# una-dinosauria/local-search-quantization

Hardware: AMD Instinct MI355X
Metric: vectors encoded/sec (ICM, m=8 h=256) (higher is better)
Workload: dtype f32

## Files before the change

local-search-quantization_amd/csrc/lsq_icmq.hip:

```cpp
#include <stdlib.h>

#include <type_traits>

#include <atomic>

#include "lsq_q16.h"
#include "lsq_xload.h"
#ifndef LSQ_WALKQ_PRIO_SHIPPED
#define LSQ_WALKQ_PRIO_SHIPPED 1
#endif
#ifdef LSQ_TUNING
__device__ unsigned long long *g_walkq_dbg = nullptr;
__device__ unsigned int g_walkq_dbg_slot = 0;
__device__ unsigned long long *g_walkq_dbg_cur = nullptr;
__device__ unsigned long long *g_walkq_blk = nullptr;
#define LSQ_WALKQ_DBG_WAVE0 (24 + 2 * 65)
#define LSQ_WALKQ_DBG_WORDS (LSQ_WALKQ_DBG_WAVE0 + 16)
#define DBG_STAMP(k) do { if (dbgp && threadIdx.x == 0) dbgp[k] = wall_clock64(); } while (0)
#define DBG_WAVE_STAMP(w) do { if (dbgp && (threadIdx.x & 63) == 0) dbgp[LSQ_WALKQ_DBG_WAVE0 + (w)] = wall_clock64(); } while (0)
#define LSQ_WALKQ_PRIO_MODE(abl) ((abl) >> 16)
#else
#define DBG_STAMP(k) do {} while (0)
#define LSQ_WALKQ_PRIO_MODE(abl) LSQ_WALKQ_PRIO_SHIPPED
#endif
// ... 217 lines not shown
        for (int k = 0; k < m; ++k) {
            if (k == j) continue;
            const double tr = (double)trange[(j * m + k) * 3] * (1.0 + 1e-6), tm = (double)trange[(j * m + k) * 3 + 1], gm = (double)trange[(j * m + k) * 3 + 2];
            rsum += tr;
            tsum += tm;
            Gmax += gm;
            sub += 2.0 * (tm + gm) + tr;
        }
        const double smax = W + sigmax + Gmax + tsum;
        sub += (W + Gmax + sigmax) * 3.0 + 2.0 * Gmax;
        const double D = rsum / 65500.0;
        const double eps = (double)(m + 1) * smax * 5.9604644775390625e-8 * 2.0 + sub * 5.9604644775390625e-8 * 2.0;
        const double slack = (double)m * (0.5 + 1.0 / 32.0) * D + eps + 65535.0 * D * 2.384185791015625e-7;
        nd.D = (float)D;
        nd.invD = (float)(1.0 / D);
        nd.hiq = (float)fmin(floor((hiU - loU) / D), 65535.0);
        nd.slack = slack;
        const double w = 2.0 * slack / D;
        nd.window = (w < 30000.0) ? (int)w + 1 : 65535;
        if (!(D > 1e-30 && D < 1e30 && rsum == rsum && smax < 1e30)) ok = false;
        if (!(nd.invD > 1e-30f && nd.invD < 1e30f)) ok = false;
        P->node[j] = nd;
    }
    P->ok = ok ? 1 : 0;
    P->nflag = 0;
}

template <int SLQ>
__global__ __launch_bounds__(256) void tables_to_q16_slices_kernel(const float *__restrict__ T, uint16_t *__restrict__ Tq, int m,
                                                                   const lsq_q16_params *__restrict__ P, const float *__restrict__ rowmin,
                                                                   const float *__restrict__ colmean) {
    constexpr int NS = LSQ_H / SLQ, LPV = SLQ / 8;
    const int64_t total = (int64_t)m * NS * (m - 1) * LSQ_H * LPV;
    const int64_t e = (int64_t)blockIdx.x * 256 + threadIdx.x;
    if (e >= total) return;
    const int qq = (int)(e % LPV);
    int64_t r = e / LPV;
    const int b = (int)(r % LSQ_H); r /= LSQ_H;
    const int kk = (int)(r % (m - 1)); r /= (m - 1);
    const int slice = (int)(r % NS);
    const int j = (int)(r / NS);
    const int k = kk + (kk >= j ? 1 : 0);
    const float lo = rowmin[((int64_t)j * m + k) * LSQ_H + b], inv = P->node[j].invD;
    const float *src = T + (((int64_t)j * m + k) * LSQ_H + b) * LSQ_H + slice * SLQ + qq * 8;
    const float *gs = colmean + ((int64_t)j * m + k) * LSQ_H + slice * SLQ + qq * 8;
    uint32_t w[4];
#pragma unroll
    for (int t = 0; t < 4; ++t) {
        const float q0 = fminf(fmaxf(rintf(((src[2 * t] - gs[2 * t]) - lo) * inv), 0.0f), 65535.0f);
        const float q1 = fminf(fmaxf(rintf(((src[2 * t + 1] - gs[2 * t + 1]) - lo) * inv), 0.0f), 65535.0f);
        w[t] = (uint32_t)q0 | ((uint32_t)q1 << 16);
    }
    const int64_t dst = (((int64_t)j * NS + slice) * (m - 1) * LSQ_H + q16_row_index<SLQ>(m, kk, b)) * LPV + qq;
    reinterpret_cast<u32x4 *>(Tq)[dst] = (u32x4){w[0], w[1], w[2], w[3]};
}

template <int M>
__device__ inline int q16_refine(const float *__restrict__ U, const uint16_t *__restrict__ Uq, const uint16_t *__restrict__ Tq,
                                 const float *__restrict__ T, uint8_t *__restrict__ rec, unsigned short *__restrict__ valid,
                                 const uint8_t *__restrict__ ref_rec, const unsigned short *__restrict__ ref_valid, int64_t n, int j,
                                 int64_t lo, const unsigned short *list, const uint32_t *arec, int namb, int SLF, int abl, unsigned short *vmir) {
    using RT = WalkqRot<M>;
    constexpr int CS = (M <= 8) ? 8 : 16;
    constexpr int RW = CS / 4;
    constexpr int AREC = 2 + RW;
    if (abl & 4) return 0;
    constexpr int NS = LSQ_H / RT::SLQ;
    constexpr int TAB = (M - 1) * LSQ_H * (RT::SLQ / 8);
    constexpr int NW = RT::NT / 64;
    const int lane = threadIdx.x & 63, wave = threadIdx.x >> 6;
    const int grp = lane >> 4, t16 = lane & 15;
    const int sl = (16 * t16) / RT::SLQ, off = (16 * t16) % RT::SLQ;
    const uint16_t *__restrict__ Uqj = Uq + (int64_t)j * n * LSQ_H;
    const uint16_t *__restrict__ Tqj = Tq + ((int64_t)j * NS + sl) * TAB * 8 + off;
    const float *__restrict__ Tj = T + (int64_t)j * M * LSQ_H * LSQ_H;
    const bool have_ref = ref_rec && ref_valid;
    int nexact = 0;
    for (int r0 = wave * 4; r0 < namb; r0 += NW * 4) {
        const int r = r0 + grp;
        const bool act = r < namb;
        const uint32_t *ar = arec + (act ? r : r0) * AREC;
        const uint32_t key = ar[0], limit = ar[1];
        uint32_t rw[RW];
#pragma unroll
        for (int w2 = 0; w2 < RW; ++w2) rw[w2] = ar[2 + w2];
        const int ci = (int)(key & 0xffffu), a1 = (int)((key >> 16) & 0xffu), a2 = (int)(key >> 24);
        const int64_t i = lo + (RT::LHOLE ? list[((ci >> 4) << 7) + (ci & 15)] : list[ci]);
        const u32x4 *up = reinterpret_cast<const u32x4 *>(Uqj + ((int64_t)sl * n + ((abl & 2) ? (int64_t)0 : i)) * RT::SLQ + off);
        u32x4 s0 = (u32x4){0xffffffffu, 0xffffffffu, 0xffffffffu, 0xffffffffu}, s1 = s0;
        if (!(abl & 8)) { s0 = up[0]; s1 = up[1]; }
        unsigned short vo = 0, rv = 0;
        uint32_t rr[RW];
#pragma unroll
        for (int w2 = 0; w2 < RW; ++w2) rr[w2] = 0;
        if (t16 == 0) {
            if (valid) vo = valid[i];
            if (have_ref) {
#pragma unroll
                for (int w2 = 0; w2 < RW; ++w2) rr[w2] = reinterpret_cast<const uint32_t *>(ref_rec + i * CS)[w2];
                rv = ref_valid[i];
            }
        }
        float term = 0.0f;
        if (M <= 8) {
            const int cand = (t16 < 8) ? a1 : a2, tt = t16 & 7;
            if (abl & 1) term = 1.0f;
            else if (tt == 0) term = U[(int64_t)j * n * LSQ_H + ((int64_t)(cand / SLF) * n + ((abl & 16) ? lo : i)) * SLF + (cand % SLF)];
            else if (tt < M) {
                const int k = (tt - 1) + ((tt - 1) >= j ? 1 : 0);
                const uint32_t bk = (rw[k >> 2] >> (8 * (k & 3))) & 0xffu;
                term = Tj[((int64_t)(k * LSQ_H) + bk) * LSQ_H + cand];
            }
        }
#pragma unroll
        for (int kk = 0; kk < M - 1; ++kk) {
            if (abl & 8) break;
            const int k = kk + (kk >= j ? 1 : 0);
            const uint32_t bk = (rw[k >> 2] >> (8 * (k & 3))) & 0xffu;
            const u32x4 *tp = reinterpret_cast<const u32x4 *>(Tqj + (int64_t)q16_row_index<RT::SLQ>(M, kk, (int)bk) * RT::SLQ);
            const u32x4 b0 = tp[0], b1 = tp[1];
            s0.x = pk_add_u16(s0.x, b0.x); s0.y = pk_add_u16(s0.y, b0.y); s0.z = pk_add_u16(s0.z, b0.z); s0.w = pk_add_u16(s0.w, b0.w);
            s1.x = pk_add_u16(s1.x, b1.x); s1.y = pk_add_u16(s1.y, b1.y); s1.z = pk_add_u16(s1.z, b1.z); s1.w = pk_add_u16(s1.w, b1.w);
        }
        uint32_t mask = 0;
#define LSQ_SURV(W, B) mask |= (((W) & 0xffffu) <= limit ? 1u : 0u) << (B); mask |= (((W) >> 16) <= limit ? 1u : 0u) << ((B) + 1);
        LSQ_SURV(s0.x, 0) LSQ_SURV(s0.y, 2) LSQ_SURV(s0.z, 4) LSQ_SURV(s0.w, 6) LSQ_SURV(s1.x, 8) LSQ_SURV(s1.y, 10) LSQ_SURV(s1.z, 12) LSQ_SURV(s1.w, 14)
#undef LSQ_SURV
        if (!act) mask = 0;
        float bv = __builtin_inff();
        int bi = 0x7fffffff;
        if (M <= 8) {
            float e = __shfl(term, (lane & ~7), 64);
#pragma unroll
            for (int q = 1; q < M; ++q) e = e + __shfl(term, (lane & ~7) + q, 64);
            const float e1 = __shfl(e, lane & ~15, 64), e2 = __shfl(e, (lane & ~15) + 8, 64);
            if (a1 / 16 == t16) mask &= ~(1u << (a1 % 16));
            if (a2 / 16 == t16) mask &= ~(1u << (a2 % 16));
            bv = e1; bi = a1;
            if (e2 < bv || (e2 == bv && a2 < bi)) { bv = e2; bi = a2; }
            if (act && t16 == 0) nexact += 2;
        }
        while (mask) {
            const int a = 16 * t16 + __builtin_ctz(mask);
            mask &= mask - 1;
            const float ev = q16_exact_value<M, RW>(U, T, n, SLF, j, i, rw, a);
            ++nexact;
            if (ev < bv || (ev == bv && a < bi)) { bv = ev; bi = a; }
        }
#pragma unroll
        for (int o = 8; o > 0; o >>= 1) {
            const float ov = __shfl_xor(bv, o, 16);
            const int oi = __shfl_xor(bi, o, 16);
            if (ov < bv || (ov == bv && oi < bi)) { bv = ov; bi = oi; }
        }
        if (act && t16 == 0) {
            const uint8_t c8 = (uint8_t)bi;
            const uint8_t old = (uint8_t)(rw[j >> 2] >> (8 * (j & 3)));
            if (c8 != old) store_code<CS>(rec, i, j, c8, rw);
            if (valid) {
                unsigned short vm = (c8 != old) ? (unsigned short)(1u << j) : (unsigned short)(vo | (1u << j));
                if (have_ref) {
                    bool same = true;
#pragma unroll
                    for (int w2 = 0; w2 < RW; ++w2) {
                        uint32_t mine = rw[w2];
                        if (w2 == (j >> 2)) mine = (mine & ~(0xffu << (8 * (j & 3)))) | ((uint32_t)c8 << (8 * (j & 3)));
                        same = same && (mine == rr[w2]);
                    }
                    if (same) vm = (unsigned short)(vm | rv);
                }
                valid[i] = vm;
                if (vmir) vmir[i - lo] = vm;
            }
        }
    }
    return nexact;
}

constexpr int WALKQ_MISC_BYTES = (20 + LSQ_WALK_COUNTERS) * 4;

template <int M>
__global__ __launch_bounds__(WalkqRot<M>::NT) __attribute__((amdgpu_waves_per_eu(4, 4))) void icm_walkq_kernel(const float *__restrict__ U, const uint16_t *__restrict__ Uq, const uint16_t *__restrict__ Tq,
                                                       const float *__restrict__ T, uint8_t *__restrict__ rec, unsigned short *__restrict__ valid,
                                                       int64_t n, const WalkNodes nodes, int per_pass, int use_skip, int direct_max,
                                                       unsigned long long *__restrict__ active_total,
                                                       const uint8_t *__restrict__ ref_rec, const unsigned short *__restrict__ ref_valid,
                                                       const lsq_q16_params *__restrict__ P, int SLF, const unsigned short *__restrict__ qflag, int abl,
                                                       const unsigned *__restrict__ gate) {
    using RT = WalkqRot<M>;
    constexpr int CS = (M <= 8) ? 8 : 16;
    constexpr int NS = LSQ_H / RT::SLQ;
    constexpr int LPV = RT::SLQ / 8;
    constexpr int VPW = 64 / LPV;
    constexpr int CW = (M - 1 + 3) / 4;
    constexpr int RW = CS / 4;
    constexpr int TAB = (M - 1) * LSQ_H * LPV;
    constexpr int PP = RT::pp();
    if (P->ok == 0) return;
    if (gate && *gate != 2u) return;
    extern __shared__ u32x4 lds_walkq[];
    constexpr int MAIN_BYTES = RT::lds_bytes();
    int *misc = reinterpret_cast<int *>(reinterpret_cast<char *>(lds_walkq) + MAIN_BYTES);
#ifdef LSQ_TUNING
    unsigned long long *dbgp = nullptr;
    if (g_walkq_dbg) {
        unsigned &dbg_slot_s = reinterpret_cast<unsigned *>(misc)[19];
        if (threadIdx.x == 0) dbg_slot_s = (blockIdx.x == 0) ? atomicAdd(&g_walkq_dbg_slot, 1u) : 0u;
        __syncthreads();
        if (blockIdx.x == 0 && dbg_slot_s < 4096) dbgp = g_walkq_dbg + (size_t)dbg_slot_s * LSQ_WALKQ_DBG_WORDS;
    }
    DBG_STAMP(0);
    if (blockIdx.x == 0 && threadIdx.x == 0) g_walkq_dbg_cur = dbgp;
    if (g_walkq_blk && threadIdx.x == 0) g_walkq_blk[2 * blockIdx.x] = wall_clock64();
#endif
    if ((uint32_t)(uintptr_t)(lds_char *)lds_walkq != 0u) __builtin_trap();
    if (LSQ_WALKQ_PRIO_MODE(abl) & 4) __builtin_amdgcn_s_setprio(3);
    u32x4 *tab = lds_walkq;
    constexpr bool HOLE = RT::HOLE;
    constexpr bool LHOLE = RT::LHOLE;
    constexpr bool ROT8 = M <= 8, ROT16 = M > 8;
    constexpr int TABE = RT::TAB_BYTES / 16;
    uint32_t *bestA = HOLE ? reinterpret_cast<uint32_t *>(reinterpret_cast<char *>(lds_walkq) + RT::HOLE_BYTE0)
                           : reinterpret_cast<uint32_t *>(lds_walkq + TABE);
    uint32_t *bestB = HOLE ? reinterpret_cast<uint32_t *>(lds_walkq + TABE) : bestA + PP;
    unsigned short *list = LHOLE ? reinterpret_cast<unsigned short *>(reinterpret_cast<char *>(lds_walkq) + RT::HOLE_BYTE0)
                                 : reinterpret_cast<unsigned short *>(bestB + PP);
    auto listp = [&](int i) -> unsigned short * { return LHOLE ? list + ((i >> 4) << 7) + (i & 15) : list + i; };
    constexpr bool MIRROR = RT::mirror();
    auto keyA = [&](int ci) -> uint32_t * { return HOLE ? bestA + ((ci >> 4) << 6) + (ci & 15) : bestA + ci; };
    auto f32slot = [&](int i) -> unsigned short * { return reinterpret_cast<unsigned short *>(keyA(i >> 1)) + (i & 1); };
    unsigned short *vmir = (MIRROR && valid) ? list + PP : nullptr;
    int *wave_tot = misc;
    int &nact_s = misc[16];
    int &redo_s = misc[17];
    int &f32_s = misc[18];
    unsigned *stat_s = reinterpret_cast<unsigned *>(misc) + 20;
    for (int e = threadIdx.x; e < LSQ_WALK_COUNTERS; e += RT::NT) stat_s[e] = 0u;
    __syncthreads();

    const int lane = threadIdx.x & 63;
    const int wave = __builtin_amdgcn_readfirstlane((int)(threadIdx.x >> 6));
    const int v = lane / LPV, q = lane % LPV;
    constexpr int NW = RT::NT / 64;
    constexpr int EPT = 4096 / RT::NT;
    constexpr int step = NW * VPW;

    struct Item { u32x4 u; uint32_t r[RW]; };

    auto walk_slices = [&](const int j, const int64_t lo, const int nact, const bool dense) {
#ifndef LSQ_TUNING
        unsigned long long *dbgp = nullptr; (void)dbgp;
#endif
        const uint16_t *__restrict__ Uqj = Uq + (int64_t)j * n * LSQ_H;
        const uint16_t *__restrict__ Tqj = Tq + (int64_t)j * NS * TAB * 8;
        uint32_t sel[CW > 0 ? CW : 1];
#pragma unroll
        for (int w = 0; w < CW; ++w) {
            uint32_t sv = 0;
#pragma unroll
            for (int t = 0; t < 4; ++t) {
                const int kk = 4 * w + t;
                const int k = kk + (kk >= j ? 1 : 0);
                sv |= (uint32_t)((kk < M - 1 ? k - 4 * w : 0) & 7) << (8 * t);
            }
            sel[w] = sv;
        }
        constexpr int NST = (TAB + RT::NT - 1) / RT::NT;
        u32x4 nxt[NST > 0 ? NST : 1];
        uint32_t selC0 = 0x0c0c0c0cu, selC1 = 0x0c0c0c0cu, base0 = 0u, base1 = 0x01000000u;
        uint32_t rotA = 0x0c0c0c0cu, rotB = 0x0c0c0c0cu, rot1A = 0x0c0c0c0cu, rot1B = 0x0c0c0c0cu, b0a = 0u, b0b = 0u, b1a = 0u, b1b = 0u;
        if constexpr (ROT16) {
#pragma unroll
            for (int t = 0; t < 8; ++t) {
                if (t < RT::NT0) {
                    const uint32_t slot = (uint32_t)(t + v) % (uint32_t)RT::NT0;
                    const uint32_t ab = ((slot << 5) | ((uint32_t)q << 4)) << (8 * (t & 3));
                    if (t < 4) { rotA = (rotA & ~(0xffu << (8 * t))) | (slot << (8 * t)); b0a |= ab; }
                    else { rotB = (rotB & ~(0xffu << (8 * (t - 4)))) | (slot << (8 * (t - 4))); b0b |= ab; }
                }
                if (t < RT::NT1) {
                    const uint32_t slot = (uint32_t)(t + v) % (uint32_t)(RT::NT1 ? RT::NT1 : 1);
                    const uint32_t ab = ((slot << 5) + (((uint32_t)q + 1u) << 4)) << (8 * (t & 3));
                    if (t < 4) { rot1A = (rot1A & ~(0xffu << (8 * t))) | (slot << (8 * t)); b1a |= ab; }
                    else { rot1B = (rot1B & ~(0xffu << (8 * (t - 4)))) | (slot << (8 * (t - 4))); b1b |= ab; }
                }
            }
        }
        if constexpr (ROT8) {
#pragma unroll
            for (int t = 0; t < RT::NT0; ++t) {
                const uint32_t slot = (uint32_t)(t + v) % (uint32_t)(RT::NT0 ? RT::NT0 : 1);
                const uint32_t k = slot + (slot >= (uint32_t)j ? 1u : 0u);
                selC0 = (selC0 & ~(0xffu << (8 * t))) | (k << (8 * t));
                base0 |= ((slot << 6) | ((uint32_t)q << 4)) << (8 * t);
            }
#pragma unroll
            for (int t = 0; t < RT::NT1; ++t) {
                const uint32_t slot = (uint32_t)(t + v) % (uint32_t)(RT::NT1 ? RT::NT1 : 1);
                const uint32_t k = 4u + slot + (4u + slot >= (uint32_t)j ? 1u : 0u);
                selC1 = (selC1 & ~(0xffu << (8 * t))) | (k << (8 * t));
                base1 |= ((slot << 6) | ((uint32_t)q << 4)) << (8 * t);
            }
        }
        const uint32_t v4 = (uint32_t)v * 4u;
        constexpr uint32_t LIST_BYTE0 = (uint32_t)(LHOLE ? 0 : RT::TAB_BYTES + PP * RT::KEY_BYTES);
        const int limv = q == 0 ? nact - v : -0x7fffffff;
        auto rot_entry = [&](auto R_) -> int {
            constexpr int r = decltype(R_)::value;
            constexpr int g = r * RT::NT >= RT::G0_ENTRIES ? 1 : 0, nt = g ? RT::NT1 : RT::NT0, e0 = r * RT::NT - g * RT::G0_ENTRIES;
            const int eg = e0 + (int)threadIdx.x;
            if constexpr (nt == RT::SPL) return g * 4096 + eg;
            else { const int code = eg / (RT::EPS * (nt ? nt : 1)); return g * 4096 + code * 16 + (eg - code * RT::EPS * nt); }
        };
        auto prefetch_tab = [&](int sl) {
            const u32x4 *src = reinterpret_cast<const u32x4 *>(Tqj) + (int64_t)sl * TAB;
#pragma unroll
            for (int r = 0; r < NST; ++r) {
                const int e = (int)threadIdx.x + r * RT::NT;
                nxt[r] = (e < TAB) ? src[e] : (u32x4){0u, 0u, 0u, 0u};
            }
        };
        prefetch_tab(0);
        const int prio = LSQ_WALKQ_PRIO_MODE(abl);
        const int wslot = (prio & 8) ? NW - 1 - wave : wave;
        const int ipw = (wslot * VPW < nact) ? (nact - wslot * VPW + step - 1) / step : 0;
        const int ipw_u = (prio & 3) ? __builtin_amdgcn_readfirstlane(ipw) : 0;
        const int h1 = (ipw_u + 3) >> 2, h2 = (ipw_u + 1) >> 1, h3 = (3 * ipw_u + 3) >> 2;
        auto item_prio = [&](int t) {
            const int tu = __builtin_amdgcn_readfirstlane(t);
            if ((prio & 3) == 1 || (prio & 3) == 3) {
                if (tu < h1) __builtin_amdgcn_s_setprio(3);
                else if (tu < h2) __builtin_amdgcn_s_setprio(2);
                else if (tu < h3) __builtin_amdgcn_s_setprio(1);
                else __builtin_amdgcn_s_setprio(0);
            } else if ((prio & 3) == 2) {
                if (tu < h2) __builtin_amdgcn_s_setprio(1);
                else __builtin_amdgcn_s_setprio(0);
            } else if (prio & 4) __builtin_amdgcn_s_setprio(0);
        };
        auto fixed_prio = [&]() {
            if (prio & 4) __builtin_amdgcn_s_setprio(3);
            else if (prio & 3) __builtin_amdgcn_s_setprio(0);
        };
        int ls = 0, lit = 0;
        const char *ub = reinterpret_cast<const char *>(Uqj + lo * RT::SLQ);
        const char *const rb = reinterpret_cast<const char *>(rec + lo * CS);
        const int64_t plane_bytes = n * (int64_t)(RT::SLQ * 2);
        auto load_next = [&](Item &it) {
            int ci = wslot * VPW + lit * step + v;
            ci = ci < nact ? ci : nact - 1;
            uint32_t li = (uint32_t)ci;
            if (!dense) {
                if constexpr (!LHOLE) li = *reinterpret_cast<lds_u16 *>(LIST_BYTE0 + 2u * (uint32_t)ci);
                else li = *listp(ci);
            }
#ifdef LSQ_TUNING
            const uint32_t uo = ((abl & 32) ? (li & 63u) : li) * (uint32_t)(RT::SLQ * 2) + (uint32_t)q * 16u;
#else
            const uint32_t uo = li * (uint32_t)(RT::SLQ * 2) + (uint32_t)q * 16u;
#endif
            it.u = __builtin_nontemporal_load(reinterpret_cast<const u32x4 *>(ub + uo));
#ifdef LSQ_TUNING
            const uint32_t *rp = reinterpret_cast<const uint32_t *>(rb + ((abl & 512) ? (li & 63u) : li) * (uint32_t)CS);
#else
            const uint32_t *rp = reinterpret_cast<const uint32_t *>(rb + li * (uint32_t)CS);
#endif
#pragma unroll
            for (int w = 0; w < RW; ++w) it.r[w] = rp[w];
            if (++lit >= ipw) {
                lit = 0;
                if (++ls < NS) ub += plane_bytes;
            }
        };
        auto compute = [&](const Item &cur, int slice, int c0) {
            u32x4 s = cur.u;
            if constexpr (ROT16) {
                uint32_t dw[4] = {0u, 0u, 0u, 0u};
#pragma unroll
                for (int w = 0; w < CW; ++w) dw[w] = __builtin_amdgcn_perm((w + 1 < RW) ? cur.r[w + 1] : 0u, cur.r[w], sel[w]);
                const uint32_t cw4[4] = {__builtin_amdgcn_perm(dw[1], dw[0], rotA), __builtin_amdgcn_perm(dw[1], dw[0], rotB),
                                         __builtin_amdgcn_perm(dw[3], dw[2], rot1A), __builtin_amdgcn_perm(dw[3], dw[2], rot1B)};
                const uint32_t bw4[4] = {b0a, b0b, b1a, b1b};
#pragma unroll
                for (int g4 = 0; g4 < 4; ++g4) {
                    const int cnt = g4 < 2 ? (RT::NT0 - 4 * g4 < 4 ? RT::NT0 - 4 * g4 : 4) : (RT::NT1 - 4 * (g4 - 2) < 4 ? RT::NT1 - 4 * (g4 - 2) : 4);
                    if (cnt <= 0) continue;
                    u32x4 rd[4];
#pragma unroll
                    for (int t = 0; t < 4; ++t)
                        if (t < cnt) {
                            const uint32_t a = __builtin_amdgcn_perm(cw4[g4], bw4[g4], 0x0c0c0400u + 0x0101u * (uint32_t)t);
                            rd[t] = *reinterpret_cast<lds_cu32x4 *>(a + (g4 < 2 ? 0u : 0xfff0u));
                        }
#ifdef LSQ_TUNING
                    if (!(abl & 64))
#endif
                    {
#pragma unroll
                        for (int t = 0; t < 4; t += 2) {
                            if (t + 1 < cnt) {
                                s.x = s.x + rd[t].x + rd[t + 1].x; s.y = s.y + rd[t].y + rd[t + 1].y;
                                s.z = s.z + rd[t].z + rd[t + 1].z; s.w = s.w + rd[t].w + rd[t + 1].w;
                            } else if (t < cnt) {
                                s.x += rd[t].x; s.y += rd[t].y; s.z += rd[t].z; s.w += rd[t].w;
                            }
                        }
                    }
                    if (g4 < 3) asm volatile("" : "+v"(s.x), "+v"(s.y), "+v"(s.z), "+v"(s.w) : : "memory");
                }
            } else {
                u32x4 rd[M > 1 ? M - 1 : 1];
                const uint32_t c0r = __builtin_amdgcn_perm(cur.r[1], cur.r[0], selC0);
#pragma unroll
                for (int t = 0; t < RT::NT0; ++t)
                    rd[t] = *reinterpret_cast<lds_cu32x4 *>(__builtin_amdgcn_perm(c0r, base0, 0x0c0c0400u + 0x0101u * (uint32_t)t));
                auto add_rows = [&](int k0, int k1) {
#ifdef LSQ_TUNING
                    if (abl & 64) return;
#endif
#pragma unroll
                    for (int kk = k0; kk < k1; kk += 2) {
                        if (kk + 1 < k1) {
                            s.x = s.x + rd[kk].x + rd[kk + 1 < M - 1 ? kk + 1 : kk].x; s.y = s.y + rd[kk].y + rd[kk + 1 < M - 1 ? kk + 1 : kk].y;
                            s.z = s.z + rd[kk].z + rd[kk + 1 < M - 1 ? kk + 1 : kk].z; s.w = s.w + rd[kk].w + rd[kk + 1 < M - 1 ? kk + 1 : kk].w;
                        } else {
                            s.x += rd[kk].x; s.y += rd[kk].y; s.z += rd[kk].z; s.w += rd[kk].w;
                        }
                    }
                };
                if constexpr (RT::NT1 > 0) {
                    const uint32_t c1r = __builtin_amdgcn_perm(cur.r[1], cur.r[0], selC1);
                    add_rows(0, RT::NT0);
                    asm volatile("" : "+v"(s.x), "+v"(s.y), "+v"(s.z), "+v"(s.w) : : "memory");
#pragma unroll
                    for (int t = 0; t < RT::NT1; ++t)
                        rd[RT::NT0 + t] = *reinterpret_cast<lds_cu32x4 *>(__builtin_amdgcn_perm(c1r, base1, 0x0c030400u + 0x0101u * (uint32_t)t));
                    add_rows(RT::NT0, M - 1);
                } else add_rows(0, M - 1);
            }
#ifdef LSQ_TUNING
            if (abl & 128) {
                if ((q == 0) & (c0 + v < nact) & (s.x == 0x12345678u)) *keyA(c0 + v) = s.y ^ s.z;
                return;
            }
#endif
            constexpr uint32_t HI = 0xffff0000u;
            const uint32_t k0 = s.x << 16, k1 = (s.x & HI) | 1u;
            const uint32_t k2 = (s.y << 16) | 2u, k3 = (s.y & HI) | 3u;
            const uint32_t k4 = (s.z << 16) | 4u, k5 = (s.z & HI) | 5u;
            const uint32_t k6 = (s.w << 16) | 6u, k7 = (s.w & HI) | 7u;
            const uint32_t lc = umin(k6, k7), hc = umax(k6, k7);
            uint32_t l0 = umin3(k0, k1, k2), h0 = umed3(k0, k1, k2);
            const uint32_t lb = umin3(k3, k4, k5), hb = umed3(k3, k4, k5);
            top2_merge(l0, h0, lb, hb);
            top2_merge(l0, h0, lc, hc);
            const uint32_t base = (uint32_t)(RT::SLQ * slice) + 8u * (uint32_t)q;
            l0 += base; h0 += base;
            if (LPV >= 2) top2_merge(l0, h0, dpp_u32<DPP_XOR1>(l0), dpp_u32<DPP_XOR1>(h0));
            if (LPV >= 4) top2_merge(l0, h0, dpp_u32<DPP_XOR2>(l0), dpp_u32<DPP_XOR2>(h0));
            if (c0 < limv) {
                if constexpr (HOLE) {
                    const uint32_t sA = (uint32_t)__builtin_amdgcn_readfirstlane((int)((uint32_t)RT::HOLE_BYTE0 + (uint32_t)c0 * 16u));
                    const uint32_t sB = (uint32_t)__builtin_amdgcn_readfirstlane((int)((uint32_t)RT::TAB_BYTES + (uint32_t)c0 * 4u));
                    const uint32_t old = __hip_atomic_fetch_min(reinterpret_cast<lds_u32 *>(sA + v4), l0, __ATOMIC_RELAXED, __HIP_MEMORY_SCOPE_WORKGROUP);
                    __hip_atomic_fetch_min(reinterpret_cast<lds_u32 *>(sB + v4), umin(umax(old, l0), h0), __ATOMIC_RELAXED, __HIP_MEMORY_SCOPE_WORKGROUP);
                } else {
                    const uint32_t old = atomicMin(&bestA[c0 + v], l0);
                    atomicMin(&bestB[c0 + v], umin(umax(old, l0), h0));
                }
            }
        };
        Item buf[RT::DEPTH];
#pragma unroll
        for (int e = 0; e < RT::DEPTH; ++e) load_next(buf[e]);
        int phase = 0;
        for (int slice = 0; slice < NS; ++slice) {
            __syncthreads();
#ifdef LSQ_TUNING
            if (slice < 8) DBG_STAMP(3 + slice);
#endif
            static_for<NST>([&](auto R_) {
                constexpr int r = decltype(R_)::value;
                if ((r + 1) * RT::NT <= TAB || r * RT::NT + (int)threadIdx.x < TAB) tab[rot_entry(R_)] = nxt[r];
            });
            __syncthreads();
#ifdef LSQ_TUNING
            if (slice == 4) DBG_STAMP(20);
#endif
            if (slice + 1 < NS) prefetch_tab(slice + 1);
#ifdef LSQ_TUNING
            if (slice == 4) DBG_STAMP(21);
#endif
            int c0 = wslot * VPW, t = 0;
            auto run = [&](auto P_) {
                constexpr int PH = decltype(P_)::value;
                for (; t + RT::DEPTH <= ipw; t += RT::DEPTH) {
                    if ((prio & 3) != 3) item_prio(t);
#pragma unroll
                    for (int e = 0; e < RT::DEPTH; ++e) {
                        if ((prio & 3) == 3) item_prio(t + e);
                        compute(buf[(PH + e) % RT::DEPTH], slice, c0); load_next(buf[(PH + e) % RT::DEPTH]); c0 += step;
                    }
                }
#pragma unroll
                for (int e = 0; e < RT::DEPTH - 1; ++e)
                    if (t < ipw) {
                        item_prio(t);
                        compute(buf[(PH + e) % RT::DEPTH], slice, c0); load_next(buf[(PH + e) % RT::DEPTH]); c0 += step;
                        ++t; phase = (PH + e + 1) % RT::DEPTH;
                    }
            };
            bool ran = false;
            auto try_phase = [&](auto P_) {
                if constexpr (decltype(P_)::value < RT::DEPTH) {
                    if (!ran && phase == decltype(P_)::value) { run(P_); ran = true; }
                }
            };
            try_phase(std::integral_constant<int, 0>{}); try_phase(std::integral_constant<int, 1>{});
            try_phase(std::integral_constant<int, 2>{}); try_phase(std::integral_constant<int, 3>{});
            fixed_prio();
#ifdef LSQ_TUNING
            if (slice == 4) { DBG_STAMP(22); DBG_WAVE_STAMP(wave); }
#endif
        }
        __syncthreads();
    };

    constexpr int LB = LSQ_LIGHT_LB(M);
    int64_t lo_cur = 0;
    auto light_list = [&](const int j, const int count, auto pick) {
        const float *__restrict__ Usj = U + (int64_t)j * n * LSQ_H;
        const float *__restrict__ Tj = T + (int64_t)j * M * LSQ_H * LSQ_H;
        for (int r0 = wave; r0 < count; r0 += NW * LB) {
            int64_t vi[LB];
            bool on[LB];
#pragma unroll
            for (int e = 0; e < LB; ++e) {
                const int r = r0 + e * NW;
                on[e] = r < count;
                vi[e] = lo_cur + __builtin_amdgcn_readfirstlane((int)pick(on[e] ? r : r0));
            }
            light_update<M, CS, LB>(rec, valid, ref_rec, ref_valid, Usj, Tj, n, SLF, j, vi, on, lane, vmir, lo_cur);
        }
    };

    const int64_t npass = (n + per_pass - 1) / per_pass;
    for (int64_t pass = blockIdx.x; pass < npass; pass += gridDim.x) {
        const int64_t lo = pass * per_pass;
        const int64_t hi = (lo + per_pass < n) ? lo + per_pass : n;
        const int cnt = (int)(hi - lo);
        lo_cur = lo;
        if (vmir) {
            __syncthreads();
            for (int idx = (int)threadIdx.x; idx < cnt; idx += RT::NT) vmir[idx] = valid[lo + idx];
            __syncthreads();
        }
        for (int nu = 0; nu < nodes.count; ++nu) {
            const int j = nodes.j[nu];
            int tix = (int)threadIdx.x;
            asm volatile("" : "+v"(tix));
#ifdef LSQ_TUNING
            if (dbgp && threadIdx.x == 0 && pass == (int64_t)blockIdx.x && nu < 64) dbgp[24 + nu] = wall_clock64();
#endif
            {
                const int base = tix * EPT;
                int f[EPT], c = 0;
#pragma unroll
                for (int e = 0; e < EPT; ++e) {
                    const int idx = base + e;
                    f[e] = 0;
                    if (idx < cnt) f[e] = (!use_skip) || !(((vmir ? vmir[idx] : valid[lo + idx]) >> j) & 1);
                    c += f[e];
                }
                int inc = c;
#pragma unroll
                for (int off = 1; off < 64; off <<= 1) {
                    const int t = __shfl_up(inc, off, 64);
                    if (lane >= off) inc += t;
                }
                if (lane == 63) wave_tot[wave] = inc;
                DBG_STAMP(16);
                __syncthreads();
                DBG_STAMP(17);
                int wbase = 0;
                for (int w2 = 0; w2 < wave; ++w2) wbase += wave_tot[w2];
                int pos = wbase + inc - c;
#pragma unroll
                for (int e = 0; e < EPT; ++e)
                    if (f[e]) *listp(pos++) = (unsigned short)(base + e);
                if (threadIdx.x == RT::NT - 1) { nact_s = wbase + inc; redo_s = 0; f32_s = 0; }
                DBG_STAMP(18);
                __syncthreads();
            }
            const int nact = nact_s;
            DBG_STAMP(1);
#ifdef LSQ_TUNING
            if (dbgp && threadIdx.x == 0 && pass == (int64_t)blockIdx.x && nu < 64) dbgp[24 + 65 + nu] = (unsigned long long)nact;
#endif
            if (nact == 0) { __syncthreads(); continue; }
            if (threadIdx.x == 0) {
                stat_s[0] += (unsigned)nact;
                stat_s[nact <= direct_max ? 2 : 3] += 1u;
                stat_s[4 + ((nodes.pos0 + nu) & (LSQ_WALK_TRACE - 1))] += (unsigned)nact;
            }
            if (nact <= direct_max) {
                light_list(j, nact, [&](int r) { return *listp(r); });
                __syncthreads();
                continue;
            }
            for (int ci = tix; ci < nact; ci += RT::NT) { *keyA(ci) = 0xffffffffu; bestB[ci] = 0xffffffffu; }
            DBG_STAMP(2);
            walk_slices(j, lo, nact, nact == cnt);
            DBG_STAMP(11);
            const lsq_q16_node &nd = P->node[j];
            const int window = nd.window;
            constexpr int EPD = (PP + RT::NT - 1) / RT::NT;
            constexpr int AREC = 2 + RW;
            constexpr int ACAP = (PP * 4) / (AREC * 4);
            {
                int64_t vi[EPD];
                uint32_t vcode[EPD], vkey[EPD], vlim[EPD];
                bool von[EPD], vamb[EPD], vf32[EPD];
                constexpr bool ONE_TRIP = (M <= 8);
                uint32_t rw[EPD][RW], rr[EPD][RW];
                unsigned short vo[EPD], rv[EPD], fl[EPD];
                uint32_t kA[EPD], kB[EPD];
                const bool have_ref = ref_rec && ref_valid;
#pragma unroll
                for (int e = 0; e < EPD; ++e) {
                    const int ci = tix + e * RT::NT;
                    vi[e] = lo; kA[e] = 0; kB[e] = 0; vo[e] = 0; rv[e] = 0; fl[e] = 0;
#pragma unroll
                    for (int w2 = 0; w2 < RW; ++w2) { rw[e][w2] = 0; rr[e][w2] = 0; }
                    if (ci < nact) {
                        kA[e] = *keyA(ci); kB[e] = bestB[ci];
                        vi[e] = lo + *listp(ci);
                        fl[e] = qflag[vi[e]];
                        if constexpr (ONE_TRIP) {
#pragma unroll
                            for (int w2 = 0; w2 < RW; ++w2) rw[e][w2] = reinterpret_cast<const uint32_t *>(rec + vi[e] * CS)[w2];
                            if (valid) vo[e] = valid[vi[e]];
                            if (have_ref) {
#pragma unroll
                                for (int w2 = 0; w2 < RW; ++w2) rr[e][w2] = reinterpret_cast<const uint32_t *>(ref_rec + vi[e] * CS)[w2];
                                rv[e] = ref_valid[vi[e]];
                            }
                        }
                    }
                }
#pragma unroll
                for (int e = 0; e < EPD; ++e) {
                    const int ci = tix + e * RT::NT;
                    von[e] = false; vamb[e] = false; vf32[e] = false; vcode[e] = 0; vkey[e] = 0; vlim[e] = 0;
                    if (ci < nact) {
                        vcode[e] = kA[e] & 0xffffu;
                        vkey[e] = (uint32_t)ci | ((kA[e] & 0xffu) << 16) | ((kB[e] & 0xffu) << 24);
                        vlim[e] = (kA[e] >> 16) + (uint32_t)window;
                        vf32[e] = (fl[e] >> j) & 1;
                        vamb[e] = !vf32[e] && ((int)(kB[e] >> 16) - (int)(kA[e] >> 16) <= window);
                        von[e] = !vamb[e] && !vf32[e];
                    }
                    if constexpr (!ONE_TRIP) {
                        if (von[e] || vamb[e]) {
#pragma unroll
                            for (int w2 = 0; w2 < RW; ++w2) rw[e][w2] = reinterpret_cast<const uint32_t *>(rec + vi[e] * CS)[w2];
                        }
                        if (von[e]) {
                            if (valid) vo[e] = valid[vi[e]];
                            if (have_ref) {
#pragma unroll
                                for (int w2 = 0; w2 < RW; ++w2) rr[e][w2] = reinterpret_cast<const uint32_t *>(ref_rec + vi[e] * CS)[w2];
                                rv[e] = ref_valid[vi[e]];
                            }
                        }
                    }
                }
                __syncthreads();
                uint32_t *arec = bestB;
#pragma unroll
                for (int e = 0; e < EPD; ++e) {
                    if (von[e]) {
                        const uint8_t c8 = (uint8_t)vcode[e];
                        const uint8_t old = (uint8_t)(rw[e][j >> 2] >> (8 * (j & 3)));
                        if (c8 != old) store_code<CS>(rec, vi[e], j, c8, rw[e]);
                        if (valid) {
                            unsigned short vm = (c8 != old) ? (unsigned short)(1u << j) : (unsigned short)(vo[e] | (1u << j));
                            if (have_ref) {
                                bool same = true;
#pragma unroll
                                for (int w2 = 0; w2 < RW; ++w2) {
                                    uint32_t mine = rw[e][w2];
                                    if (w2 == (j >> 2)) mine = (mine & ~(0xffu << (8 * (j & 3)))) | ((uint32_t)c8 << (8 * (j & 3)));
                                    same = same && (mine == rr[e][w2]);
                                }
                                if (same) vm = (unsigned short)(vm | rv[e]);
                            }
                            valid[vi[e]] = vm;
                            if (vmir) vmir[vi[e] - lo] = vm;
                        }
                    }
                    bool tof32 = vf32[e];
                    if (vamb[e]) {
                        const int slot = atomicAdd(&redo_s, 1);
                        if (slot < ACAP) {
                            arec[slot * AREC] = vkey[e];
                            arec[slot * AREC + 1] = vlim[e];
#pragma unroll
                            for (int w2 = 0; w2 < RW; ++w2) arec[slot * AREC + 2 + w2] = rw[e][w2];
                        } else tof32 = true;
                    }
                    if (tof32) *f32slot(atomicAdd(&f32_s, 1)) = (unsigned short)(vkey[e] & 0xffffu);
                }
            }
            __syncthreads();
            DBG_STAMP(12);
            const int namb = redo_s < ACAP ? redo_s : ACAP;
            int nexact = q16_refine<M>(U, Uq, Tq, T, rec, valid, ref_rec, ref_valid, n, j, lo, list, bestB, namb, SLF, abl, vmir);
            {
                const int nf32 = f32_s;
                light_list(j, nf32, [&](int r) { return *listp(*f32slot(r)); });
                if (threadIdx.x == 0 && nf32) atomicAdd(&stat_s[4 + LSQ_WALK_TRACE + 2], (unsigned)nf32);
            }
            {
#pragma unroll
                for (int o = 32; o > 0; o >>= 1) nexact += __shfl_xor(nexact, o, 64);
                if (lane == 0 && nexact) atomicAdd(&stat_s[4 + LSQ_WALK_TRACE + 1], (unsigned)nexact);
                if (threadIdx.x == 0 && namb) atomicAdd(&stat_s[4 + LSQ_WALK_TRACE], (unsigned)namb);
            }
            __syncthreads();
            DBG_STAMP(13);
#ifdef LSQ_TUNING
            if (dbgp && threadIdx.x == 0) { dbgp[14] = (unsigned long long)nact; dbgp[15] = (unsigned long long)namb; }
#endif
        }
    }
    __syncthreads();
#ifdef LSQ_TUNING
    if (dbgp && threadIdx.x == 0) dbgp[24 + 64] = wall_clock64();
    if (g_walkq_blk && threadIdx.x == 0) g_walkq_blk[2 * blockIdx.x + 1] = wall_clock64();
#endif
    if (active_total)
        for (int e = threadIdx.x; e < LSQ_WALK_COUNTERS; e += RT::NT)
            if (stat_s[e]) atomicAdd(active_total + e, (unsigned long long)stat_s[e]);
}

}

#ifdef LSQ_TUNING
extern "C" __attribute__((visibility("default"))) int lsq_tuning_set_walkq_debug(void *buf) {
    unsigned zero = 0;
    LSQ_HIP(hipMemcpyToSymbol(HIP_SYMBOL(g_walkq_dbg), &buf, sizeof(buf)));
    LSQ_HIP(hipMemcpyToSymbol(HIP_SYMBOL(g_walkq_dbg_slot), &zero, sizeof(zero)));
    return LSQ_OK;
}
extern "C" __attribute__((visibility("default"))) int lsq_tuning_set_walkq_block_clock(void *buf) {
    LSQ_HIP(hipMemcpyToSymbol(HIP_SYMBOL(g_walkq_blk), &buf, sizeof(buf)));
    return LSQ_OK;
}
#endif

__global__ void q16_road_kernel(const lsq_q16_params *__restrict__ P, unsigned *__restrict__ road, long long pairs, long long fallback_div) {
    if (threadIdx.x != 0) return;
    const bool filtered = P->ok == 1 && (long long)P->nflag * fallback_div <= pairs;
    road[0] = filtered ? 2u : 0u;
    if (!filtered) road[1] += 1u;
}
__global__ void q16_probe_kernel(const unsigned long long *__restrict__ probe, unsigned long long *__restrict__ totals, unsigned *__restrict__ road,
                                 unsigned long long probe_div) {
    const int e = threadIdx.x;
    if (e < LSQ_WALK_COUNTERS && totals) totals[e] += probe[e];
    if (e == 0 && road[0] == 2u && probe_div > 0) {
        const unsigned long long hard = probe[4 + LSQ_WALK_TRACE] + probe[4 + LSQ_WALK_TRACE + 2];
        if ((double)hard * (double)probe_div > (double)probe[0]) { road[0] = 0u; road[1] += 1u; }
    }
}
int lsq_launch_q16_road(hipStream_t s, const lsq_q16_params *P, unsigned *road, int64_t pairs, int64_t fallback_div) {
    hipLaunchKernelGGL(q16_road_kernel, dim3(1), dim3(64), 0, s, P, road, (long long)pairs, (long long)fallback_div);
    LSQ_HIP(hipGetLastError());
    return LSQ_OK;
}
int lsq_launch_q16_probe(hipStream_t s, const unsigned long long *probe, unsigned long long *totals, unsigned *road, int64_t probe_div) {
    hipLaunchKernelGGL(q16_probe_kernel, dim3(1), dim3(128), 0, s, probe, totals, road, (unsigned long long)probe_div);
    LSQ_HIP(hipGetLastError());
    return LSQ_OK;
}

const void *lsq_probe_kernel_icmq() { return reinterpret_cast<const void *>(&q16_range_init_kernel); }

template <class XT>
int lsq_launch_unary_shift_panel(hipStream_t s, const XT *Xp, int64_t rows, int d, int m, const lsq_q16_work &w, int64_t row0) {
    if (rows <= 0) return LSQ_OK;
    const int64_t shift_blocks = (rows * 16 + 255) / 256;
    LSQ_SHIFT_LAUNCH(d, dim3((unsigned)(shift_blocks < 2048 ? shift_blocks : 2048)), s, Xp, w.means, rows, d, m, w.sigma + (size_t)row0 * m,
                       &w.qrange[lsq_q16_work::Q_PANEL_SINK], &w.qrange[lsq_q16_work::Q_SIGBOUND], w.qflag, row0, w.P);
    LSQ_HIP(hipGetLastError());
    return LSQ_OK;
}

template int lsq_launch_unary_shift_panel(hipStream_t, const float *, int64_t, int, int, const lsq_q16_work &, int64_t);
template int lsq_launch_unary_shift_panel(hipStream_t, const uint8_t *, int64_t, int, int, const lsq_q16_work &, int64_t);

int lsq_q16_sample_rows(int64_t n, int d, int64_t *rts_out) {
    const int64_t nsample = d <= 128 ? 16384 : (d <= 512 ? 8192 : 4096);
    const int64_t rts = n > nsample ? n / nsample : 1;
    if (rts_out) *rts_out = rts;
    return (int)((n + 128 * rts - 1) / (128 * rts));
}

template <class XT>
int lsq_launch_q16_prepare(hipStream_t s, const XT *X, int64_t n, int d, const float *K, const float *sci, const float *T, int m, const lsq_q16_work &w,
                           int tables_changed) {
    using W = lsq_q16_work;
    const XT *Xsample = static_cast<const XT *>(w.Xsample);
    unsigned *sigmax = &w.qrange[W::Q_SIGMAX];
    static_assert(W::Q_SIGBOUND == W::Q_SIGMAX + 1 && W::Q_WORDS == 2 * LSQ_MAX_M + 4, "q16_params_kernel's sigrange[0 .. 1], q16_range_init_kernel's fill");
    if (tables_changed) {
        LSQ_HIP(hipMemsetAsync(w.bad, 0, sizeof(int), s));
        hipLaunchKernelGGL(table_colmean_kernel, dim3((unsigned)(m * m)), dim3(256), 0, s, T, m, w.colmean);
        hipLaunchKernelGGL(unary_colshift_kernel, dim3((unsigned)m), dim3(256), 0, s, w.colmean, m, w.colshift);
        if (m > 1) hipLaunchKernelGGL(table_range_kernel, dim3((unsigned)(m * m)), dim3(256), 0, s, T, m, w.colmean, w.trange, w.rowmin, w.bad);
        hipLaunchKernelGGL(codebook_means_kernel, dim3((unsigned)((d + 63) / 64), (unsigned)m), dim3(256), 0, s, K, m, d, w.means);
    }
    hipLaunchKernelGGL(q16_range_init_kernel, dim3(1), dim3(64), 0, s, w.qrange, m);
    lsq_gemm_q16 range;
    range.qrange = w.qrange; range.colshift = w.colshift;
    if (Xsample) {
        const int64_t shift_blocks = (w.nsample_rows * 16 + 255) / 256;
        LSQ_SHIFT_LAUNCH(d, dim3((unsigned)(shift_blocks < 2048 ? shift_blocks : 2048)), s, Xsample, w.means, w.nsample_rows, d, m, w.sigma_sample, sigmax);
        range.sigma = w.sigma_sample;
        LSQ_TRY(lsq_launch_chain_gemm(s, Xsample, K, sci, -2.0f, w.nsample_rows, m * LSQ_H, d, LSQ_H, 0, 0, nullptr, 0, w.nsample_rows, 0, &range));
        LSQ_HIP(hipMemsetAsync(w.qflag, 0, sizeof(unsigned short) * (size_t)((n + 1) & ~(int64_t)1), s));
    } else if (n > 0) {
        const int64_t shift_blocks = (n * 16 + 255) / 256;
        LSQ_SHIFT_LAUNCH(d, dim3((unsigned)(shift_blocks < 2048 ? shift_blocks : 2048)), s, X, w.means, n, d, m, w.sigma, sigmax);
        int64_t rts64 = 1;
        (void)lsq_q16_sample_rows(n, d, &rts64);
        range.rts = (int)rts64; range.sigma = w.sigma;
        LSQ_TRY(lsq_launch_chain_gemm(s, X, K, sci, -2.0f, n, m * LSQ_H, d, LSQ_H, 0, 0, nullptr, 0, n, 0, &range));
        LSQ_HIP(hipMemsetAsync(w.qflag, 0, sizeof(unsigned short) * (size_t)((n + 1) & ~(int64_t)1), s));
    }
    hipLaunchKernelGGL(q16_params_kernel, dim3(1), dim3(64), 0, s, w.trange, w.bad, w.qrange, m, w.P, sigmax, Xsample ? 2.0f : 1.0f);
    if (m > 1) {
        const int slq = lsq_q16_slice_width(m);
        const int64_t total = (int64_t)m * (LSQ_H / slq) * (m - 1) * LSQ_H * (slq / 8);
        const unsigned grid = (unsigned)((total + 255) / 256);
        if (slq == 32) hipLaunchKernelGGL(tables_to_q16_slices_kernel<32>, dim3(grid), dim3(256), 0, s, T, w.Tq, m, w.P, w.rowmin, w.colmean);
        else hipLaunchKernelGGL(tables_to_q16_slices_kernel<16>, dim3(grid), dim3(256), 0, s, T, w.Tq, m, w.P, w.rowmin, w.colmean);
    }
    LSQ_HIP(hipGetLastError());
    return LSQ_OK;
}

template int lsq_launch_q16_prepare(hipStream_t, const float *, int64_t, int, const float *, const float *, const float *, int, const lsq_q16_work &, int);
template int lsq_launch_q16_prepare(hipStream_t, const uint8_t *, int64_t, int, const float *, const float *, const float *, int, const lsq_q16_work &, int);

template <int M>
static int launch_walkq_t(hipStream_t s, const float *U, const uint16_t *Uq, const uint16_t *Tq, const float *T, uint8_t *rec, unsigned short *valid,
                          int64_t n, const WalkNodes &nodes, int use_skip, unsigned long long *active_total, int light,
                          const uint8_t *ref_rec, const unsigned short *ref_valid, const lsq_q16_params *P, const unsigned short *qflag, const unsigned *gate) {
    using RT = WalkqRot<M>;
    constexpr int PP = RT::pp();
    constexpr int LDS_BYTES = RT::lds_bytes() + WALKQ_MISC_BYTES;
    static_assert(LDS_BYTES <= 160 * 1024 && WALKQ_MISC_BYTES <= 768, "slice table + keys must fit the 160 KiB LDS");
    constexpr int NBLK = 256;
    int per_pass = 1, npass = 1;
    lsq_walk_geometry(n, PP, &per_pass, &npass);
    const int direct_max = light >= 0 ? light : LSQ_KNOB("LSQ_WALK_DIRECT", 160);
    const int skip = (use_skip && valid) ? 1 : 0;
    static LdsOptIn optin;
    LSQ_TRY(optin_lds(optin, &icm_walkq_kernel<M>, LDS_BYTES));
    static std::atomic<int> static_lds_known{-1};
    int static_lds = static_lds_known.load(std::memory_order_relaxed);
    if (static_lds < 0) {
        hipFuncAttributes fa;
        LSQ_HIP(hipFuncGetAttributes(&fa, reinterpret_cast<const void *>(&icm_walkq_kernel<M>)));
        static_lds = (int)fa.sharedSizeBytes;
        static_lds_known.store(static_lds, std::memory_order_relaxed);
    }
    if (static_lds != 0) { lsq_set_error("icm_walkq_kernel<%d>: %d bytes of static LDS in a kernel that addresses LDS from 0", M, static_lds); return LSQ_EHIP; }
    const unsigned grid = (unsigned)(npass < NBLK ? npass : NBLK);
    hipLaunchKernelGGL((icm_walkq_kernel<M>), dim3(grid), dim3(RT::NT), LDS_BYTES, s, U, Uq, Tq, T, rec, valid, n, nodes, per_pass, skip,
                       direct_max, active_total, skip ? ref_rec : nullptr, skip ? ref_valid : nullptr, P, lsq_walk_slice_width(M), qflag,
                       LSQ_KNOB("LSQ_Q16_ABL", 0) | (LSQ_KNOB("LSQ_WALKQ_PRIO", LSQ_WALKQ_PRIO_SHIPPED) << 16), gate);
    LSQ_HIP(hipGetLastError());
    return LSQ_OK;
}

int lsq_launch_icm_walkq(hipStream_t s, const float *U, const uint16_t *Uq, const uint16_t *Tq, const float *T, uint8_t *rec, unsigned short *valid,
                         int64_t n, int m, const int32_t *order, int nnodes, int pos0, int max_per, int use_skip, unsigned long long *active_total, int light,
                         const uint8_t *ref_rec, const unsigned short *ref_valid, const lsq_q16_params *P, const unsigned short *qflag, const unsigned *gate,
                         int *launched) {
    if (n <= 0 || nnodes <= 0) return LSQ_OK;
    return for_walk_launches(order, nnodes, pos0, m, max_per, launched, [&](const WalkNodes &nodes) -> int {
        LSQ_DISPATCH_M(m, LSQ_TRY((launch_walkq_t<M_>(s, U, Uq, Tq, T, rec, valid, n, nodes, use_skip, active_total, light, ref_rec, ref_valid, P, qflag, gate))));
        return LSQ_OK;
    });
}
```

local-search-quantization_amd/csrc/lsq_q16.h:

```cpp
#pragma once

#include "lsq_wave.h"

typedef unsigned short u16x2 __attribute__((ext_vector_type(2)));
typedef unsigned int u32x4 __attribute__((ext_vector_type(4)));

namespace {

typedef const u32x4 __attribute__((address_space(3))) lds_cu32x4;
typedef uint32_t __attribute__((address_space(3))) lds_u32;
typedef const unsigned short __attribute__((address_space(3))) lds_u16;
typedef char __attribute__((address_space(3))) lds_char;


__device__ inline uint32_t pk_add_u16(uint32_t a, uint32_t b) {
    return __builtin_bit_cast(uint32_t, __builtin_bit_cast(u16x2, a) + __builtin_bit_cast(u16x2, b));
}
__device__ inline uint32_t umin(uint32_t a, uint32_t b) { return a < b ? a : b; }
__device__ inline uint32_t umax(uint32_t a, uint32_t b) { return a > b ? a : b; }
__device__ inline uint32_t umin3(uint32_t a, uint32_t b, uint32_t c) { uint32_t r; asm("v_min3_u32 %0, %1, %2, %3" : "=v"(r) : "v"(a), "v"(b), "v"(c)); return r; }
__device__ inline uint32_t umed3(uint32_t a, uint32_t b, uint32_t c) { uint32_t r; asm("v_med3_u32 %0, %1, %2, %3" : "=v"(r) : "v"(a), "v"(b), "v"(c)); return r; }
__device__ inline void top2_merge(uint32_t &lo, uint32_t &hi, uint32_t olo, uint32_t ohi) {
    const uint32_t nhi = umin3(umax(lo, olo), hi, ohi);
    lo = umin(lo, olo);
    hi = nhi;
}
template <int CTRL>
__device__ inline uint32_t dpp_u32(uint32_t v) {
    return (uint32_t)__builtin_amdgcn_update_dpp(0, (int)v, CTRL, 0xf, 0xf, true);
}


template <int M, int RW>
__device__ inline float q16_exact_value(const float *__restrict__ U, const float *__restrict__ T, int64_t n, int SLF, int j, int64_t i,
                            const uint32_t (&rw)[RW], int a) {
    float s = U[(int64_t)j * n * LSQ_H + ((int64_t)(a / SLF) * n + i) * SLF + (a % SLF)];
    const float *Tj = T + (int64_t)j * M * LSQ_H * LSQ_H;
#pragma unroll
    for (int k = 0; k < M; ++k) {
        if (k == j) continue;
        const uint32_t bk = (rw[k >> 2] >> (8 * (k & 3))) & 0xffu;
        s = s + Tj[((int64_t)(k * LSQ_H) + bk) * LSQ_H + a];
    }
    return s;
}


template <int M>
struct WalkqRot {
    static constexpr int SLQ = lsq_q16_slice_width(M);
    static constexpr int DEPTH = M <= 8 ? 3 : 2;
    static constexpr int NT = 1024;
    static constexpr int NTAB = M - 1;
    static constexpr int SPL = M <= 8 ? 4 : 8;
    static constexpr int SLOT_BYTES = 256 / SPL, EPS = SLOT_BYTES / 16;
    static constexpr int NT0 = NTAB < SPL ? NTAB : SPL, NT1 = NTAB - NT0;
    static constexpr int NG = NT1 > 0 ? 2 : (NT0 > 0 ? 1 : 0);
    static constexpr int TAB_BYTES = NG * 65536;
    static constexpr int G0_ENTRIES = NT0 * LSQ_H * EPS;
    static constexpr bool HOLE = M <= 8 && NT1 > 0;
    static constexpr bool LHOLE = M > 8 && NT1 > 0;
    static constexpr int HOLE_BYTE0 = 65536 + 256 - SLOT_BYTES;
    static constexpr int pp_for(int bytes_per_vector) {
        const int avail = 160 * 1024 - 768 - TAB_BYTES;
        const int v = avail / bytes_per_vector / 64 * 64;
        return v > 4096 ? 4096 : v;
    }
    static constexpr int KEY_BYTES = HOLE ? 4 : 8;
    static constexpr int LIST_BYTES = LHOLE ? 0 : 2;
    static constexpr bool mirror() { return M <= 8 && pp_for(KEY_BYTES + LIST_BYTES + 2) * 256 >= 1000000; }
    static constexpr int pp() { return pp_for(KEY_BYTES + LIST_BYTES + (mirror() ? 2 : 0)); }
    static constexpr int lds_bytes() { return TAB_BYTES + pp() * (KEY_BYTES + LIST_BYTES + (mirror() ? 2 : 0)); }
};

template <int N, class F, int I = 0>
__device__ inline void static_for(F &&f) {
    if constexpr (I < N) { f(std::integral_constant<int, I>{}); static_for<N, F, I + 1>(static_cast<F &&>(f)); }
}

template <int SLQ>
__host__ __device__ inline int q16_row_index(int m, int kk, int code) {
    const int spl = SLQ == 32 ? 4 : 8;
    const int nt0 = m - 1 < spl ? m - 1 : spl, g = kk >= spl ? 1 : 0;
    return g ? nt0 * LSQ_H + code * (m - 1 - nt0) + (kk - spl) : code * nt0 + kk;
}

}
```

Before: 22.16 million.

## Keep per-vector top-2 keys in registers instead of LDS atomics

Replaces the per-item LDS/global atomicMin updates of best and second-best keys with register-resident top-2 accumulators. Items are mapped to lane slots of key pairs through an exec-masked min/max sequence, and the results are written out once after all slices. This also removes the initialization pass that reset the key arrays before each walk. The cost is extra VGPRs for the key pairs and a more complex, statically unrolled item-to-slot mapping, which could lower occupancy.

```diff
diff --git a/local-search-quantization_amd/csrc/lsq_icmq.hip b/local-search-quantization_amd/csrc/lsq_icmq.hip
--- a/local-search-quantization_amd/csrc/lsq_icmq.hip
+++ b/local-search-quantization_amd/csrc/lsq_icmq.hip
@@ -543,9 +543,11 @@
                 base1 |= ((slot << 6) | ((uint32_t)q << 4)) << (8 * t);
             }
         }
-        const uint32_t v4 = (uint32_t)v * 4u;
         constexpr uint32_t LIST_BYTE0 = (uint32_t)(LHOLE ? 0 : RT::TAB_BYTES + PP * RT::KEY_BYTES);
-        const int limv = q == 0 ? nact - v : -0x7fffffff;
+        static_assert(PP <= 4096 && RT::KNB * RT::KBLK >= RT::MAXI && RT::KPAIRS * LPV >= RT::MAXI, "every item of a wave needs a lane slot of a key pair");
+        uint32_t kl[RT::KPAIRS], kh[RT::KPAIRS];
+#pragma unroll
+        for (int p = 0; p < RT::KPAIRS; ++p) { kl[p] = 0xffffffffu; kh[p] = 0xffffffffu; }
         auto rot_entry = [&](auto R_) -> int {
             constexpr int r = decltype(R_)::value;
             constexpr int g = r * RT::NT >= RT::G0_ENTRIES ? 1 : 0, nt = g ? RT::NT1 : RT::NT0, e0 = r * RT::NT - g * RT::G0_ENTRIES;
@@ -613,7 +615,8 @@
                 if (++ls < NS) ub += plane_bytes;
             }
         };
-        auto compute = [&](const Item &cur, int slice, int c0) {
+        auto compute = [&](const Item &cur, int slice, auto KP_, uint64_t klanes) {
+            constexpr int KP = decltype(KP_)::value;
             u32x4 s = cur.u;
             if constexpr (ROT16) {
                 uint32_t dw[4] = {0u, 0u, 0u, 0u};
@@ -681,7 +684,7 @@
             }
 #ifdef LSQ_TUNING
             if (abl & 128) {
-                if ((q == 0) & (c0 + v < nact) & (s.x == 0x12345678u)) *keyA(c0 + v) = s.y ^ s.z;
+                if (s.x == 0x12345678u) kl[KP] = s.y ^ s.z;
                 return;
             }
 #endif
@@ -699,17 +702,7 @@
             l0 += base; h0 += base;
             if (LPV >= 2) top2_merge(l0, h0, dpp_u32<DPP_XOR1>(l0), dpp_u32<DPP_XOR1>(h0));
             if (LPV >= 4) top2_merge(l0, h0, dpp_u32<DPP_XOR2>(l0), dpp_u32<DPP_XOR2>(h0));
-            if (c0 < limv) {
-                if constexpr (HOLE) {
-                    const uint32_t sA = (uint32_t)__builtin_amdgcn_readfirstlane((int)((uint32_t)RT::HOLE_BYTE0 + (uint32_t)c0 * 16u));
-                    const uint32_t sB = (uint32_t)__builtin_amdgcn_readfirstlane((int)((uint32_t)RT::TAB_BYTES + (uint32_t)c0 * 4u));
-                    const uint32_t old = __hip_atomic_fetch_min(reinterpret_cast<lds_u32 *>(sA + v4), l0, __ATOMIC_RELAXED, __HIP_MEMORY_SCOPE_WORKGROUP);
-                    __hip_atomic_fetch_min(reinterpret_cast<lds_u32 *>(sB + v4), umin(umax(old, l0), h0), __ATOMIC_RELAXED, __HIP_MEMORY_SCOPE_WORKGROUP);
-                } else {
-                    const uint32_t old = atomicMin(&bestA[c0 + v], l0);
-                    atomicMin(&bestB[c0 + v], umin(umax(old, l0), h0));
-                }
-            }
+            top2_keep(kl[KP], kh[KP], l0, h0, klanes);
         };
         Item buf[RT::DEPTH];
 #pragma unroll
@@ -732,24 +725,43 @@
 #ifdef LSQ_TUNING
             if (slice == 4) DBG_STAMP(21);
 #endif
-            int c0 = wslot * VPW, t = 0;
+            int t = 0;
+            auto step_item = [&](Item &it, auto KP_, uint64_t klanes) { compute(it, slice, KP_, klanes); load_next(it); };
             auto run = [&](auto P_) {
                 constexpr int PH = decltype(P_)::value;
-                for (; t + RT::DEPTH <= ipw; t += RT::DEPTH) {
-                    if ((prio & 3) != 3) item_prio(t);
-#pragma unroll
-                    for (int e = 0; e < RT::DEPTH; ++e) {
-                        if ((prio & 3) == 3) item_prio(t + e);
-                        compute(buf[(PH + e) % RT::DEPTH], slice, c0); load_next(buf[(PH + e) % RT::DEPTH]); c0 += step;
+                static_for<RT::KNB>([&](auto B_) {
+                    constexpr int b = decltype(B_)::value, T0 = b * RT::KBLK;
+                    if constexpr (RT::knarrow(b)) {
+                        if (ipw > T0) {
+#pragma unroll
+                            for (int e = 0; e < RT::MAXI - T0; ++e)
+                                if (T0 + e < ipw) {
+                                    item_prio(T0 + e);
+                                    step_item(buf[(PH + e) % RT::DEPTH], std::integral_constant<int, b * RT::DEPTH>{}, RT::KLANES0 << e);
+                                    phase = (PH + e + 1) % RT::DEPTH;
+                                }
+                        }
+                    } else {
+                        const int lim = ipw < T0 + RT::KBLK ? ipw : T0 + RT::KBLK;
+                        uint64_t kslot = RT::KLANES0;
+                        for (; t + RT::DEPTH <= lim; t += RT::DEPTH, kslot <<= 1) {
+                            if ((prio & 3) != 3) item_prio(t);
+                            static_for<RT::DEPTH>([&](auto E_) {
+                                constexpr int e = decltype(E_)::value;
+                                if ((prio & 3) == 3) item_prio(t + e);
+                                step_item(buf[(PH + e) % RT::DEPTH], std::integral_constant<int, b * RT::DEPTH + e>{}, kslot);
+                            });
+                        }
+                        static_for<RT::DEPTH - 1>([&](auto E_) {
+                            constexpr int e = decltype(E_)::value;
+                            if (t < lim) {
+                                item_prio(t);
+                                step_item(buf[(PH + e) % RT::DEPTH], std::integral_constant<int, b * RT::DEPTH + e>{}, kslot);
+                                ++t; phase = (PH + e + 1) % RT::DEPTH;
+                            }
+                        });
                     }
-                }
-#pragma unroll
-                for (int e = 0; e < RT::DEPTH - 1; ++e)
-                    if (t < ipw) {
-                        item_prio(t);
-                        compute(buf[(PH + e) % RT::DEPTH], slice, c0); load_next(buf[(PH + e) % RT::DEPTH]); c0 += step;
-                        ++t; phase = (PH + e + 1) % RT::DEPTH;
-                    }
+                });
             };
             bool ran = false;
             auto try_phase = [&](auto P_) {
@@ -764,6 +776,14 @@
             if (slice == 4) { DBG_STAMP(22); DBG_WAVE_STAMP(wave); }
 #endif
         }
+        int pl = lane;
+        asm volatile("" : "+v"(pl));
+#pragma unroll
+        for (int p = 0; p < RT::KPAIRS; ++p) {
+            const int ci = wslot * VPW + RT::key_item(p, pl % LPV) * step + pl / LPV;
+            if (ci < nact) { *keyA(ci) = kl[p]; bestB[ci] = kh[p]; }
+        }
+        DBG_STAMP(23);
         __syncthreads();
     };
 
@@ -849,7 +869,6 @@
                 __syncthreads();
                 continue;
             }
-            for (int ci = tix; ci < nact; ci += RT::NT) { *keyA(ci) = 0xffffffffu; bestB[ci] = 0xffffffffu; }
             DBG_STAMP(2);
             walk_slices(j, lo, nact, nact == cnt);
             DBG_STAMP(11);
diff --git a/local-search-quantization_amd/csrc/lsq_q16.h b/local-search-quantization_amd/csrc/lsq_q16.h
--- a/local-search-quantization_amd/csrc/lsq_q16.h
+++ b/local-search-quantization_amd/csrc/lsq_q16.h
@@ -24,6 +24,12 @@
     const uint32_t nhi = umin3(umax(lo, olo), hi, ohi);
     lo = umin(lo, olo);
     hi = nhi;
+}
+__device__ inline void top2_keep(uint32_t &lo, uint32_t &hi, uint32_t olo, uint32_t ohi, uint64_t lanes) {
+    uint32_t t;
+    uint64_t saved;
+    asm("s_and_saveexec_b64 %3, %6\n\tv_max_u32 %2, %0, %4\n\tv_min3_u32 %1, %2, %1, %5\n\tv_min_u32 %0, %0, %4\n\ts_mov_b64 exec, %3"
+        : "+v"(lo), "+v"(hi), "=&v"(t), "=&s"(saved) : "v"(olo), "v"(ohi), "s"(lanes) : "scc");
 }
 template <int CTRL>
 __device__ inline uint32_t dpp_u32(uint32_t v) {
@@ -71,6 +77,13 @@
     static constexpr bool mirror() { return M <= 8 && pp_for(KEY_BYTES + LIST_BYTES + 2) * 256 >= 1000000; }
     static constexpr int pp() { return pp_for(KEY_BYTES + LIST_BYTES + (mirror() ? 2 : 0)); }
     static constexpr int lds_bytes() { return TAB_BYTES + pp() * (KEY_BYTES + LIST_BYTES + (mirror() ? 2 : 0)); }
+    static constexpr int LPV = SLQ / 8, VPW = 64 / LPV;
+    static constexpr int MAXI = (4096 + (NT / 64) * VPW - 1) / ((NT / 64) * VPW);
+    static constexpr uint64_t KLANES0 = LPV == 4 ? 0x1111111111111111ull : 0x5555555555555555ull;
+    static constexpr int KBLK = DEPTH * LPV, KNB = (MAXI + KBLK - 1) / KBLK;
+    static constexpr bool knarrow(int b) { return b == KNB - 1 && MAXI - b * KBLK <= LPV; }
+    static constexpr int KPAIRS = (KNB - 1) * DEPTH + (knarrow(KNB - 1) ? 1 : DEPTH);
+    static constexpr int key_item(int p, int q) { return knarrow(p / DEPTH) ? (p / DEPTH) * KBLK + q : (p / DEPTH) * KBLK + q * DEPTH + p % DEPTH; }
 };
 
 template <int N, class F, int I = 0>
```

After: 21.83 million. -1.5%, worse.
